# deepqmc/deepqmc

Hardware: AMD Instinct MI355X
Metric: walker*local-energy evals/sec (VMC step: n_sub Metropolis sub-steps + E_loc + energy reduction) (higher is better)
Workload: dtype f32

## Files before the change

deepqmc_amd/csrc/kernel_linear.hip:

```cpp
#include "common.h"
#include "kernels.h"

namespace dqmc {

template <typename real> __device__ __forceinline__ void act_derivs(int act, real v, real& y, real& d1, real& d2) {
  if (act == 1) {
    y = r_tanh<real>(v);
    d1 = 1 - y * y;
    d2 = -2 * y * d1;
  } else if (act == 2) {
    const real s = 1 / (1 + r_exp<real>(-v));
    y = v * s;
    d1 = s * (1 + v * (1 - s));
    d2 = s * (1 - s) * (2 + v * (1 - 2 * s));
  } else if (act == 3) {
    const real av = v < 0 ? -v : v;
    const real e = r_exp<real>(-av);
    const real s = v >= 0 ? 1 / (1 + e) : e / (1 + e);
    y = (v > 0 ? v : (real)0) + (sizeof(real) == 4 ? (real)log1pf((float)e) : (real)log1p((double)e)) - (real)0.69314718055994530942;
    d1 = s;
    d2 = s * (1 - s);
  } else if (act == 4) {
    const real t = r_tanh<real>(v * (real)0.25);
    y = 1 + 2 * t;
// ... 146 lines not shown
        sink.rows(m_ok[q] ? m : 0, drow[q], rrow[q]);
      }
      real rres[2][NR], rpre[2][NR];
#pragma unroll
      for (int q = 0; q < 2; ++q)
#pragma unroll
        for (int n = 0; n < NR; ++n) {
          const int col = col_w0 + n * 16 + cl;
          rres[q][n] = sink.fetch_at(rrow[q], col, col_ok[n] && m_ok[q]);
          rpre[q][n] = (pre != nullptr && col_ok[n]) ? pre[(long)b[q] * ld_pre + col] : (real)0;
        }
#pragma unroll
      for (int q = 0; q < 2; ++q) {
        const int tile_row = wm * (16 * MR) + i * 16 + Mfma<real>::row_of(lane, r0 + q);
#pragma unroll
        for (int n = 0; n < NR; ++n) {
          const int col = col_w0 + n * 16 + cl;
          real v = acc[i][n][r0 + q];
          if (pre != nullptr && col_ok[n]) v += rpre[q][n];
          if (bias != nullptr && col_ok[n]) v += bv[n];
          sink.put_at(drow[q], tile_row, col, act_value<real, ACT>(v), rres[q][n], col_ok[n] && m_ok[q]);
        }
      }
    }
}

template <typename real, int MR, int NR, int GPW, typename Sink>
__device__ __forceinline__ void lin_epilogue(typename Mfma<real>::acc_t (&acc)[MR][NR], const LinArgs<real>& a, const real* bias, int act,
                                             int ldw, const real* pre, int col_w0, int wm, int n_groups, Sink& sink, int bx,
                                             real* xch = nullptr) {
  constexpr bool HALF = GPW == -1;
  constexpr bool SPLIT = GPW == -2;
  constexpr int GB = GPW > 0 ? MR / GPW : 1;
  const int lane = threadIdx.x & 63, cl = lane & 15;
  if (HALF) {
    constexpr bool F32L = sizeof(real) == 4;
    const int wmu = __builtin_amdgcn_readfirstlane(wm);
    const int Tm1 = a.T - 1;
    const int q = lane >> 4;
    real bvh[NR];
    bool col_ok[NR];
#pragma unroll
    for (int n = 0; n < NR; ++n) {
      const int col = col_w0 + n * 16 + cl;
      col_ok[n] = col < ldw;
      bvh[n] = (bias != nullptr && col_ok[n]) ? bias[col] : (real)0;
    }
#pragma unroll
    for (int i = 0; i < MR; ++i) {
      const int g0 = ((bx * 4 + wmu) * MR + i) * 2;
      const bool ok0 = g0 < n_groups, ok1 = g0 + 1 < n_groups;
      if (!ok0) {
        if constexpr (Sink::fills) {
          sink.ugroup2(0, false, col_w0);
#pragma unroll
          for (int n = 0; n < NR; ++n)
#pragma unroll
            for (int rg = 0; rg < 4; ++rg) sink.uput2(false, 0, wm * (16 * MR) + i * 16 + Mfma<real>::row_of(lane, rg), n * 16 + cl, (real)0, (real)0);
        }
        continue;
      }
      sink.ugroup2(g0, ok1, col_w0);
      real rres[NR][4];
#pragma unroll
      for (int n = 0; n < NR; ++n)
#pragma unroll
        for (int rg = 0; rg < 4; ++rg) {
          const int row = Mfma<real>::row_of(lane, rg);
          const bool h = row >> 3;
          rres[n][rg] = (col_ok[n] && (!h || ok1)) ? sink.ufetch2(h, row & 7, n * 16 + cl) : (real)0;
        }
#pragma unroll
      for (int n = 0; n < NR; ++n) {
        real y[2], d1[2], d2S[2];
        if constexpr (F32L) {
          real v = __shfl(acc[i][n][0], (lane & 32) + cl, 64) + bvh[n];
          real s_part = 0;
#pragma unroll
          for (int rg = 0; rg < 4; ++rg) {
            const int tt = (4 * q + rg) & 7;
            const real x = acc[i][n][rg];
            if (tt > 0 && tt < Tm1) s_part += x * x;
          }
          const real S = s_part + __shfl_xor(s_part, 16, 64);
          real d2;
          act_derivs<real>(act, v, y[0], d1[0], d2);
          d2S[0] = d2 * S;
          y[1] = y[0]; d1[1] = d1[0]; d2S[1] = d2S[0];
        } else {
#pragma unroll
          for (int h = 0; h < 2; ++h) {
            const real v = __shfl(acc[i][n][2 * h], cl, 64) + bvh[n];
            real s_part = 0;
#pragma unroll
            for (int rg = 2 * h; rg < 2 * h + 2; ++rg) {
              const int tt = Mfma<real>::row_of(lane, rg) & 7;
              const real x = acc[i][n][rg];
              if (tt > 0 && tt < Tm1) s_part += x * x;
            }
            const real S = quad_sum<real>(s_part);
            real d2;
            act_derivs<real>(act, v, y[h], d1[h], d2);
            d2S[h] = d2 * S;
          }
        }
#pragma unroll
        for (int rg = 0; rg < 4; ++rg) {
          const int row = Mfma<real>::row_of(lane, rg), tt = row & 7;
          const bool h = row >> 3;
          const int hs_ = F32L ? 0 : (rg >> 1);
          const real x = acc[i][n][rg];
          real o = r_fma<real>(d1[hs_], x, tt == Tm1 ? d2S[hs_] : (real)0);
          if (tt == 0) o = y[hs_];
          if (tt > Tm1) o = 0;
          const bool ok = col_ok[n] && (!h || ok1);
          if constexpr (Sink::fills) sink.uput2(h, tt, wm * (16 * MR) + i * 16 + row, n * 16 + cl, ok ? o : (real)0, rres[n][rg]);
          else if (ok) sink.uput2(h, tt, wm * (16 * MR) + i * 16 + row, n * 16 + cl, o, rres[n][rg]);
        }
      }
    }
  } else if (SPLIT) {
    const int half = wm & 1, gl = wm >> 1;
    const int g = bx * 2 + gl;
    const bool g_ok = g < n_groups;
    const int b = (g_ok ? g : 0) / a.nrows;
    const int t0 = half * (16 * MR);
    sink.group(0, g_ok ? g : 0);
    if (pre != nullptr && g_ok) {
#pragma unroll
      for (int n = 0; n < NR; ++n) {
        const int col = col_w0 + n * 16 + cl;
        if (col < ldw) {
#pragma unroll
          for (int tb = 0; tb < MR; ++tb)
#pragma unroll
            for (int rg = 0; rg < 4; ++rg) {
              const int t = t0 + tb * 16 + Mfma<real>::row_of(lane, rg);
              acc[tb][n][rg] += pre[((long)b * a.TP + t) * a.ld_pre + col];
            }
        }
      }
    }
    real* xv = xch + gl * (3 * NR * 16);
    real* xs = xv + NR * 16;
    __syncthreads();
#pragma unroll
    for (int n = 0; n < NR; ++n) {
      real s_part = 0;
#pragma unroll
      for (int tb = 0; tb < MR; ++tb)
#pragma unroll
        for (int rg = 0; rg < 4; ++rg) {
          const int t = t0 + tb * 16 + Mfma<real>::row_of(lane, rg);
          const real x = acc[tb][n][rg];
          if (t >= 1 && t < a.T - 1) s_part += x * x;
        }
      const real Sh = quad_sum<real>(s_part);
      if (lane < 16) {
        xs[half * (NR * 16) + n * 16 + cl] = Sh;
        if (half == 0) xv[n * 16 + cl] = acc[0][n][0];
      }
    }
    __syncthreads();
#pragma unroll
    for (int n = 0; n < NR; ++n) {
      const int col = col_w0 + n * 16 + cl;
      const bool col_ok = col < ldw;
      real v = xv[n * 16 + cl];
      if (bias != nullptr && col_ok) v += bias[col];
      const real S = xs[n * 16 + cl] + xs[NR * 16 + n * 16 + cl];
      real rres[MR][4];
#pragma unroll
      for (int tb = 0; tb < MR; ++tb)
#pragma unroll
        for (int rg = 0; rg < 4; ++rg) rres[tb][rg] = sink.fetch(0, t0 + tb * 16 + Mfma<real>::row_of(lane, rg), col, col_ok && g_ok);
      real y, d1, d2;
      act_derivs<real>(act, v, y, d1, d2);
#pragma unroll
      for (int tb = 0; tb < MR; ++tb)
#pragma unroll
        for (int rg = 0; rg < 4; ++rg) {
          const int row = Mfma<real>::row_of(lane, rg);
          const int t = t0 + tb * 16 + row;
          const real x = acc[tb][n][rg];
          real o;
          if (t == 0) o = y;
          else if (t < a.T - 1) o = d1 * x;
          else if (t == a.T - 1) o = d1 * x + d2 * S;
          else o = 0;
          sink.put(0, t, wm * (16 * MR) + tb * 16 + row, col, o, rres[tb][rg], col_ok && g_ok);
        }
    }
  } else if (GPW > 0) {
    constexpr int NG = GPW > 0 ? GPW : 1;
    constexpr bool HOIST = GB * NR * 4 * (int)(sizeof(real) / 4) <= 32;
    const int wmu = __builtin_amdgcn_readfirstlane(wm);
    const int Tm1 = a.T - 1;
    real bv[NR];
    bool col_ok[NR];
#pragma unroll
    for (int n = 0; n < NR; ++n) {
      const int col = col_w0 + n * 16 + cl;
      col_ok[n] = col < ldw;
      bv[n] = (bias != nullptr && col_ok[n]) ? bias[col] : (real)0;
    }
#pragma unroll
    for (int gj = 0; gj < NG; ++gj) {
      const int g = (bx * 4 + wmu) * GPW + gj;
      if (g >= n_groups) {
        if constexpr (Sink::fills) {
          sink.ugroup(0, col_w0);
#pragma unroll
          for (int n = 0; n < NR; ++n)
#pragma unroll
            for (int tb = 0; tb < GB; ++tb)
#pragma unroll
              for (int rg = 0; rg < 4; ++rg)
                sink.uput(0, wm * (16 * MR) + (gj * GB + tb) * 16 + Mfma<real>::row_of(lane, rg), n * 16 + cl, (real)0, (real)0);
        }
        continue;
      }
      sink.ugroup(g, col_w0);
      if (pre != nullptr) {
        const real* pw = pre + uniform_off((long)(g / a.nrows) * a.TP * a.ld_pre + col_w0);
#pragma unroll
        for (int n = 0; n < NR; ++n) {
          if (col_ok[n]) {
#pragma unroll
            for (int tb = 0; tb < GB; ++tb)
#pragma unroll
              for (int rg = 0; rg < 4; ++rg) {
                const int t = tb * 16 + Mfma<real>::row_of(lane, rg);
                acc[gj * GB + tb][n][rg] += *reinterpret_cast<const real*>(reinterpret_cast<const char*>(pw) + (unsigned)((t * a.ld_pre + n * 16 + cl) * (int)sizeof(real)));
              }
          }
        }
      }
      real rall[HOIST ? NR : 1][HOIST ? GB : 1][4];
      if constexpr (HOIST) {
#pragma unroll
        for (int n = 0; n < NR; ++n)
#pragma unroll
          for (int tb = 0; tb < GB; ++tb)
#pragma unroll
            for (int rg = 0; rg < 4; ++rg)
              rall[n][tb][rg] = col_ok[n] ? sink.ufetch(tb * 16 + Mfma<real>::row_of(lane, rg), n * 16 + cl) : (real)0;
      }
#pragma unroll
      for (int n = 0; n < NR; ++n) {
        real v = __shfl(acc[gj * GB][n][0], cl, 64) + bv[n];
        real s_part = 0;
#pragma unroll
        for (int tb = 0; tb < GB; ++tb)
#pragma unroll
          for (int rg = 0; rg < 4; ++rg) {
            const int t = tb * 16 + Mfma<real>::row_of(lane, rg);
            const real x = acc[gj * GB + tb][n][rg];
            if (t >= 1 && t < Tm1) s_part += x * x;
          }
        const real S = quad_sum<real>(s_part);
        real y, d1, d2;
        act_derivs<real>(act, v, y, d1, d2);
        const real d2S = d2 * S;
        constexpr int FB = HOIST ? GB : (((sizeof(real) == 8 && GB > 2) || GB == 4) ? 2 : GB);
#pragma unroll
        for (int tb0 = 0; tb0 < GB; tb0 += FB) {
          real rres[FB][4];
#pragma unroll
          for (int tb = 0; tb < FB; ++tb)
#pragma unroll
            for (int rg = 0; rg < 4; ++rg) {
              if constexpr (HOIST) rres[tb][rg] = rall[n][tb][rg];
              else rres[tb][rg] = (tb0 + tb < GB && col_ok[n]) ? sink.ufetch((tb0 + tb) * 16 + Mfma<real>::row_of(lane, rg), n * 16 + cl) : (real)0;
            }
          if (Sink::fills || col_ok[n]) {
#pragma unroll
            for (int tb = tb0; tb < tb0 + FB && tb < GB; ++tb)
#pragma unroll
              for (int rg = 0; rg < 4; ++rg) {
                const int row = Mfma<real>::row_of(lane, rg);
                const int t = tb * 16 + row;
                const real x = acc[gj * GB + tb][n][rg];
                real o = r_fma<real>(d1, x, t == Tm1 ? d2S : (real)0);
                if (t == 0) o = y;
                if (t > Tm1) o = 0;
                if (Sink::fills && !col_ok[n]) o = 0;
                sink.uput(t, wm * (16 * MR) + (gj * GB + tb) * 16 + row, n * 16 + cl, o, rres[tb - tb0][rg]);
              }
          }
        }
      }
    }
  } else {
    switch (act) {
      case 1: value_rows_epilogue<real, MR, NR, 1>(acc, a.nrows, a.ld_pre, bias, ldw, pre, col_w0, wm, n_groups, sink, bx); break;
      case 2: value_rows_epilogue<real, MR, NR, 2>(acc, a.nrows, a.ld_pre, bias, ldw, pre, col_w0, wm, n_groups, sink, bx); break;
      case 3: value_rows_epilogue<real, MR, NR, 3>(acc, a.nrows, a.ld_pre, bias, ldw, pre, col_w0, wm, n_groups, sink, bx); break;
      case 4: value_rows_epilogue<real, MR, NR, 4>(acc, a.nrows, a.ld_pre, bias, ldw, pre, col_w0, wm, n_groups, sink, bx); break;
      default: value_rows_epilogue<real, MR, NR, 0>(acc, a.nrows, a.ld_pre, bias, ldw, pre, col_w0, wm, n_groups, sink, bx); break;
    }
  }
}

template <typename real, int MR, int NR, int GPW, int WN, bool CHAIN = false, int NR2 = 2, int BKX = 1>
__global__ void __launch_bounds__(256 * WN, GPW == -2 ? 2 : (GPW == 0 && NR == 4 && WN == 2 && MR * sizeof(real) == 16) ? 4 : 1) k_linear(const LinArgs<real> a) {
  constexpr int NT = 256 * WN;
  constexpr int BM = 64 * MR, BN = 16 * NR * WN, BK = 16 * BKX, BK2 = 16;
  constexpr int AS = BK + 2, BS = BStride<BN>::v;
  constexpr bool HALF = GPW == -1;
  constexpr bool SPLIT = GPW == -2;
  constexpr int GB = GPW > 0 ? MR / GPW : 1;
  constexpr int APT = MR / WN;
  constexpr int NBV = (BK * BN / 4 + NT - 1) / NT;
  constexpr int HS = CHAIN ? BN + 2 : 1;
  constexpr int BN2 = 16 * NR2, BS2 = BStride<BN2>::v;
  constexpr bool FRESH = sizeof(real) == 4 && GPW != 0 && MR <= 3;
  static_assert(MR % WN == 0, "MR must be a multiple of WN");
  static_assert(!CHAIN || WN == 1, "chained layers use one column tile");
  static_assert(!SPLIT || (!CHAIN && WN == 1 && 6 * NR * 16 <= BM * AS), "split groups: plain layers, one column tile per workgroup");
  typedef typename Mfma<real>::acc_t acc_t;
  constexpr int N_AB = BM * AS + BK * BS, N_H = CHAIN ? BM * HS : 0, N_MAIN = N_AB > N_H ? N_AB : N_H;
  __shared__ __attribute__((aligned(32))) real smem_lin[N_MAIN + (CHAIN ? BK2 * BS2 : 0)];
  real* const As = smem_lin;
  real* const Bs = smem_lin + BM * AS;
  real* const Hs = smem_lin;
  real* const Bs2 = smem_lin + N_MAIN;
  static_assert((BM * AS) % 4 == 0 && N_MAIN % 4 == 0, "16-byte (float) / 32-byte (double) aligned LDS tiles");

  const int tid = threadIdx.x, lane = tid & 63, wave = tid >> 6;
  const int wm = wave & 3, wn = wave >> 2;
  const int n_groups = a.B * a.nrows;
  const TileId tile = tile_of_block();
  const int bx = tile.bx;
  const int col_blk0 = tile.by * BN;

  int a_row[APT];
  int a_g[APT], a_t[APT];
  const int a_kq = tid & 3;
#pragma unroll
  for (int j = 0; j < APT; ++j) {
    const int row = (tid >> 2) + (NT / 4) * j;
    a_row[j] = row;
    int g, t;
    if (HALF) {
      const int w = row / (16 * MR), rb = (row >> 4) % MR;
      g = ((bx * 4 + w) * MR + rb) * 2 + ((row & 15) >> 3);
      t = row & 7;
    } else if (SPLIT) {
      const int w = row / (16 * MR), rb = (row >> 4) % MR;
      g = bx * 2 + (w >> 1);
      t = ((w & 1) * MR + rb) * 16 + (row & 15);
    } else if (GPW > 0) {
      const int w = row / (16 * MR), rb = (row >> 4) % MR;
      g = (bx * 4 + w) * GPW + rb / GB;
      t = (rb % GB) * 16 + (row & 15);
    } else {
      g = bx * BM + row;
      t = 0;
    }
    a_g[j] = g < n_groups ? g : -1;
    a_t[j] = t;
  }

  acc_t acc[MR][NR];
#pragma unroll
  for (int i = 0; i < MR; ++i)
#pragma unroll
    for (int j = 0; j < NR; ++j) acc[i][j] = acc_t{0, 0, 0, 0};

  for (int p = 0; p < a.n_pieces; ++p) {
    const LinPiece<real> pc = a.piece[p];
    const int w_row0 = pc.w_row;
    const real* a_src[APT];
#pragma unroll
    for (int j = 0; j < APT; ++j) {
      if (a_g[j] >= 0) {
        const int b = a_g[j] / a.nrows, rr = a_g[j] - b * a.nrows;
        const long srow = ((long)b * pc.rpw + pc.r0 + (pc.bcast ? 0 : rr)) * a.TP + a_t[j];
        a_src[j] = pc.src + srow * pc.ld;
      } else {
        a_src[j] = nullptr;
      }
    }
    const int n_chunks = (pc.K + BK - 1) / BK;
    Vec4<real> ra[APT][BKX];
    real rb_[NBV][4];
    auto load_chunk = [&](int kc) {
#pragma unroll
      for (int j = 0; j < APT; ++j)
#pragma unroll
        for (int x = 0; x < BKX; ++x) {
          const int k0 = kc * BK + 16 * x + 4 * a_kq;
          if (a_src[j] != nullptr && k0 < pc.K) ra[j][x] = *reinterpret_cast<const Vec4<real>*>(a_src[j] + k0);
          else ra[j][x] = Vec4<real>{{0, 0, 0, 0}};
        }
#pragma unroll
      for (int j = 0; j < NBV; ++j) {
        const int f = tid + NT * j;
        const int k = f / (BN / 4), n4 = f % (BN / 4);
        const int kk = kc * BK + k, col = col_blk0 + 4 * n4;
        Vec4<real> t{{0, 0, 0, 0}};
        if (f < BK * BN / 4 && kk < pc.K && col < a.ldw) t = *reinterpret_cast<const Vec4<real>*>(a.W + (long)(w_row0 + kk) * a.ldw + col);
#pragma unroll
        for (int x = 0; x < 4; ++x) rb_[j][x] = t.v[x];
      }
    };
    load_chunk(0);
    for (int kc = 0; kc < n_chunks; ++kc) {
      __syncthreads();
#pragma unroll
      for (int j = 0; j < APT; ++j)
#pragma unroll
        for (int x = 0; x < BKX; ++x) {
          Vec2<real>* dst = reinterpret_cast<Vec2<real>*>(&As[a_row[j] * AS + 16 * x + 4 * a_kq]);
          dst[0] = Vec2<real>{{ra[j][x].v[0], ra[j][x].v[1]}};
          dst[1] = Vec2<real>{{ra[j][x].v[2], ra[j][x].v[3]}};
        }
#pragma unroll
      for (int j = 0; j < NBV; ++j) {
        const int f = tid + NT * j;
        if (f < BK * BN / 4) {
          const int k = f / (BN / 4), n4 = f % (BN / 4);
          *reinterpret_cast<Vec4<real>*>(&Bs[k * BS + 4 * n4]) = Vec4<real>{{rb_[j][0], rb_[j][1], rb_[j][2], rb_[j][3]}};
        }
      }
      __syncthreads();
      if (kc + 1 < n_chunks) load_chunk(kc + 1);
      acc_t part[FRESH ? MR : 1][FRESH ? NR : 1];
      if (FRESH) {
#pragma unroll
        for (int i = 0; i < MR; ++i)
#pragma unroll
          for (int j = 0; j < NR; ++j) part[FRESH ? i : 0][FRESH ? j : 0] = acc_t{0, 0, 0, 0};
      }
#pragma unroll
      for (int kk = 0; kk < BK / 4; ++kk) {
        const int kcol = kk * 4 + (lane >> 4);
        real fa[MR], fb[NR];
#pragma unroll
        for (int i = 0; i < MR; ++i) fa[i] = As[(wm * (16 * MR) + i * 16 + (lane & 15)) * AS + kcol];
#pragma unroll
        for (int j = 0; j < NR; ++j) fb[j] = Bs[kcol * BS + wn * (16 * NR) + j * 16 + (lane & 15)];
#pragma unroll
        for (int i = 0; i < MR; ++i)
#pragma unroll
          for (int j = 0; j < NR; ++j) {
            if (FRESH) part[FRESH ? i : 0][FRESH ? j : 0] = Mfma<real>::run(fa[i], fb[j], part[FRESH ? i : 0][FRESH ? j : 0]);
            else acc[i][j] = Mfma<real>::run(fa[i], fb[j], acc[i][j]);
          }
      }
      if (FRESH) {
#pragma unroll
        for (int i = 0; i < MR; ++i)
#pragma unroll
          for (int j = 0; j < NR; ++j)
#pragma unroll
            for (int x = 0; x < 4; ++x) acc[i][j][x] += part[FRESH ? i : 0][FRESH ? j : 0][x];
      }
    }
  }

  if (!CHAIN) {
    HbmSink<real> sink(a);
    lin_epilogue<real, MR, NR, GPW>(acc, a, a.bias, a.act, a.ldw, a.pre, col_blk0 + wn * (16 * NR), wm, n_groups, sink, bx, As);
    return;
  }
  auto second_layer = [&](acc_t (&h)[MR][NR], const real* bias1, const real* W2, const real* bias2, const LinArgs<real>& out) {
    static_assert(BK2 * BN2 / 4 <= NT, "one W2 vector per thread and chunk");
    const int K2 = a.ldw;
    const int n_chunks2 = (K2 + BK2 - 1) / BK2;
    real w2r[NR][4];
#pragma unroll
    for (int kc = 0; kc < NR; ++kc) {
      const int k = tid / (BN2 / 4), n4 = tid % (BN2 / 4);
      const int kk = kc * BK2 + k, col = 4 * n4;
      Vec4<real> t{{0, 0, 0, 0}};
      if (tid < BK2 * BN2 / 4 && kc < n_chunks2 && kk < K2 && col < a.ldw2) t = *reinterpret_cast<const Vec4<real>*>(W2 + (long)kk * a.ldw2 + col);
#pragma unroll
      for (int x = 0; x < 4; ++x) w2r[kc][x] = t.v[x];
    }
    {
      __syncthreads();
      LdsSink<real> hsink{Hs, HS};
      lin_epilogue<real, MR, NR, GPW>(h, a, bias1, a.act, a.ldw, (const real*)nullptr, 0, wm, n_groups, hsink, bx);
    }
    acc_t acc2[MR][NR2];
#pragma unroll
    for (int i = 0; i < MR; ++i)
#pragma unroll
      for (int j = 0; j < NR2; ++j) acc2[i][j] = acc_t{0, 0, 0, 0};
#pragma unroll
    for (int kc = 0; kc < NR; ++kc) {
      if (kc < n_chunks2) {
      __syncthreads();
      if (tid < BK2 * BN2 / 4) {
        const int k = tid / (BN2 / 4), n4 = tid % (BN2 / 4);
        *reinterpret_cast<Vec4<real>*>(&Bs2[k * BS2 + 4 * n4]) = Vec4<real>{{w2r[kc][0], w2r[kc][1], w2r[kc][2], w2r[kc][3]}};
      }
      __syncthreads();
#pragma unroll
      for (int kk = 0; kk < 4; ++kk) {
        const int kcol = kk * 4 + (lane >> 4);
        real fa[MR], fb[NR2];
#pragma unroll
        for (int i = 0; i < MR; ++i) fa[i] = Hs[(wm * (16 * MR) + i * 16 + (lane & 15)) * HS + kc * BK2 + kcol];
#pragma unroll
        for (int j = 0; j < NR2; ++j) fb[j] = Bs2[kcol * BS2 + j * 16 + (lane & 15)];
#pragma unroll
        for (int i = 0; i < MR; ++i)
#pragma unroll
          for (int j = 0; j < NR2; ++j) acc2[i][j] = Mfma<real>::run(fa[i], fb[j], acc2[i][j]);
      }
      }
    }
    HbmSink<real> sink(out);
    lin_epilogue<real, MR, NR2, GPW>(acc2, out, bias2, a.act2, a.ldw2, (const real*)nullptr, 0, wm, n_groups, sink, bx);
  };
  second_layer(acc, a.bias, a.W2, a.bias2, a);
}

__device__ __forceinline__ void sched_fence() { __builtin_amdgcn_sched_barrier(0); }
template <int MR, int NR, int GPW, int WN, int NP>
__global__ void __launch_bounds__(256 * WN, (MR == 3 && WN == 1) ? 3 : 1) k_linear_bf(const LinArgs<float> a) {
  typedef float real;
  constexpr int NT = 256 * WN;
  constexpr int BM = 64 * MR, BN = 16 * NR * WN, BK = 32;
  constexpr int AS = BK + 2, BSTR = BN + 4;
  constexpr bool HALF = GPW == -1;
  constexpr int GB = GPW > 0 ? MR / GPW : 1;
  constexpr int APT = MR / WN;
  constexpr int NBI = ((BK / 2) * (BN / 4) + NT - 1) / NT;
  constexpr bool HOLD_A = MR <= NR;
  constexpr bool BF_FRESH = NP == 9;
  static_assert(MR % WN == 0, "MR must be a multiple of WN");
  typedef Mfma<float>::acc_t acc_t;
  HIP_DYNAMIC_SHARED(char, smem_raw)
  float* As = reinterpret_cast<float*>(smem_raw);
  uint32_t* Bs = reinterpret_cast<uint32_t*>(smem_raw + (size_t)BM * AS * 4);

  const int tid = threadIdx.x, lane = tid & 63, wave = tid >> 6;
  const int wm = wave & 3, wn = wave >> 2;
  const int n_groups = a.B * a.nrows;
  const TileId tile = tile_of_block();
  const int bx = tile.bx;
  const int col_blk0 = tile.by * BN;
  const int kg = lane >> 4, l15 = lane & 15;

  int a_row[APT], a_g[APT], a_t[APT];
  const int a_kq = tid & 3;
#pragma unroll
  for (int j = 0; j < APT; ++j) {
    const int row = (tid >> 2) + (NT / 4) * j;
    a_row[j] = row;
    int g, t;
    if (HALF) {
      const int w = row / (16 * MR), rb = (row >> 4) % MR;
      g = ((bx * 4 + w) * MR + rb) * 2 + ((row & 15) >> 3);
      t = row & 7;
    } else if (GPW > 0) {
      const int w = row / (16 * MR), rb = (row >> 4) % MR;
      g = (bx * 4 + w) * GPW + rb / GB;
      t = (rb % GB) * 16 + (row & 15);
    } else {
      g = bx * BM + row;
      t = 0;
    }
    a_g[j] = g < n_groups ? g : -1;
    a_t[j] = t;
  }

  acc_t acc[MR][NR];
#pragma unroll
  for (int i = 0; i < MR; ++i)
#pragma unroll
    for (int j = 0; j < NR; ++j) acc[i][j] = acc_t{0, 0, 0, 0};

  for (int p = 0; p < a.n_pieces; ++p) {
    const LinPiece<real> pc = a.piece[p];
    const int w_row0 = pc.w_row;
    const real* a_src[APT];
#pragma unroll
    for (int j = 0; j < APT; ++j) {
      if (a_g[j] >= 0) {
        const int b = a_g[j] / a.nrows, rr = a_g[j] - b * a.nrows;
        const long srow = ((long)b * pc.rpw + pc.r0 + (pc.bcast ? 0 : rr)) * a.TP + a_t[j];
        a_src[j] = pc.src + srow * pc.ld;
      } else {
        a_src[j] = nullptr;
      }
    }
    const int n_chunks = (pc.K + BK - 1) / BK;
    Vec4<real> ra[APT][2], rb_[NBI][2];
    auto load_chunk = [&](int kc) {
#pragma unroll
      for (int j = 0; j < APT; ++j)
#pragma unroll
        for (int x = 0; x < 2; ++x) {
          const int k0 = kc * BK + 16 * x + 4 * a_kq;
          if (a_src[j] != nullptr && k0 < pc.K) ra[j][x] = *reinterpret_cast<const Vec4<real>*>(a_src[j] + k0);
          else ra[j][x] = Vec4<real>{{0, 0, 0, 0}};
        }
#pragma unroll
      for (int j = 0; j < NBI; ++j) {
        const int f = tid + NT * j;
        const int kp = f / (BN / 4), n4 = f % (BN / 4);
        const int kk = kc * BK + 2 * kp, col = col_blk0 + 4 * n4;
#pragma unroll
        for (int h = 0; h < 2; ++h) {
          if (f < (BK / 2) * (BN / 4) && kk + h < pc.K && col < a.ldw)
            rb_[j][h] = *reinterpret_cast<const Vec4<real>*>(a.W + (long)(w_row0 + kk + h) * a.ldw + col);
          else
            rb_[j][h] = Vec4<real>{{0, 0, 0, 0}};
        }
      }
    };
    load_chunk(0);
    for (int kc = 0; kc < n_chunks; ++kc) {
      __syncthreads();
#pragma unroll
      for (int j = 0; j < APT; ++j)
#pragma unroll
        for (int x = 0; x < 2; ++x) {
          Vec2<real>* dst = reinterpret_cast<Vec2<real>*>(&As[a_row[j] * AS + 16 * x + 4 * a_kq]);
          dst[0] = Vec2<real>{{ra[j][x].v[0], ra[j][x].v[1]}};
          dst[1] = Vec2<real>{{ra[j][x].v[2], ra[j][x].v[3]}};
        }
#pragma unroll
      for (int j = 0; j < NBI; ++j) {
        const int f = tid + NT * j;
        if (f < (BK / 2) * (BN / 4)) {
          const int kp = f / (BN / 4), n4 = f % (BN / 4);
          BfFrag* d0 = reinterpret_cast<BfFrag*>(&Bs[(0 * 16 + kp) * BSTR + 4 * n4]);
          BfFrag* d1 = reinterpret_cast<BfFrag*>(&Bs[(1 * 16 + kp) * BSTR + 4 * n4]);
          BfFrag* d2 = reinterpret_cast<BfFrag*>(&Bs[(2 * 16 + kp) * BSTR + 4 * n4]);
          uint32_t w0[4], w1[4], w2[4];
#pragma unroll
          for (int c = 0; c < 4; ++c) {
            const float x0 = rb_[j][0].v[c], x1 = rb_[j][1].v[c];
            const uint32_t h = bf_pack2(x0, x1);
            const float r0 = x0 - bf_lo_as_float(h), r1 = x1 - bf_hi_as_float(h);
            const uint32_t m = bf_pack2(r0, r1);
            w0[c] = h; w1[c] = m; w2[c] = bf_pack2(r0 - bf_lo_as_float(m), r1 - bf_hi_as_float(m));
          }
          *d0 = BfFrag{{w0[0], w0[1], w0[2], w0[3]}};
          *d1 = BfFrag{{w1[0], w1[1], w1[2], w1[3]}};
          *d2 = BfFrag{{w2[0], w2[1], w2[2], w2[3]}};
        }
      }
      __syncthreads();
      if (kc + 1 < n_chunks) load_chunk(kc + 1);
      auto read_a = [&](int i, BfFrag& p0, BfFrag& p1, BfFrag& p2) {
        float av[8];
        const Vec2<real>* src = reinterpret_cast<const Vec2<real>*>(&As[(wm * (16 * MR) + i * 16 + l15) * AS + 8 * kg]);
#pragma unroll
        for (int q = 0; q < 4; ++q) { const Vec2<real> t = src[q]; av[2 * q] = t.v[0]; av[2 * q + 1] = t.v[1]; }
        bf_split8(av, p0, p1, p2);
      };
      auto read_b = [&](int j, BfFrag& p0, BfFrag& p1, BfFrag& p2) {
        const int col = wn * (16 * NR) + j * 16 + l15;
#pragma unroll
        for (int q = 0; q < 4; ++q) {
          p0.w[q] = Bs[(0 * 16 + 4 * kg + q) * BSTR + col];
          p1.w[q] = Bs[(1 * 16 + 4 * kg + q) * BSTR + col];
          p2.w[q] = Bs[(2 * 16 + 4 * kg + q) * BSTR + col];
        }
      };
      if (HOLD_A) {
        BfFrag fa[MR][3];
#pragma unroll
        for (int i = 0; i < MR; ++i) read_a(i, fa[i][0], fa[i][1], fa[i][2]);
#pragma unroll
        for (int j = 0; j < NR; ++j) {
          BfFrag b0, b1, b2;
          read_b(j, b0, b1, b2);
          acc_t part[MR];
#pragma unroll
          for (int i = 0; i < MR; ++i) part[i] = BF_FRESH ? acc_t{0, 0, 0, 0} : acc[i][j];
          if (NP == 9) {
#pragma unroll
            for (int i = 0; i < MR; ++i) part[i] = mfma_bf16(fa[i][2], b2, part[i]);
#pragma unroll
            for (int i = 0; i < MR; ++i) part[i] = mfma_bf16(fa[i][2], b1, part[i]);
#pragma unroll
            for (int i = 0; i < MR; ++i) part[i] = mfma_bf16(fa[i][1], b2, part[i]);
          }
#pragma unroll
          for (int i = 0; i < MR; ++i) part[i] = mfma_bf16(fa[i][2], b0, part[i]);
#pragma unroll
          for (int i = 0; i < MR; ++i) part[i] = mfma_bf16(fa[i][1], b1, part[i]);
#pragma unroll
          for (int i = 0; i < MR; ++i) part[i] = mfma_bf16(fa[i][0], b2, part[i]);
#pragma unroll
          for (int i = 0; i < MR; ++i) part[i] = mfma_bf16(fa[i][1], b0, part[i]);
#pragma unroll
          for (int i = 0; i < MR; ++i) part[i] = mfma_bf16(fa[i][0], b1, part[i]);
#pragma unroll
          for (int i = 0; i < MR; ++i) part[i] = mfma_bf16(fa[i][0], b0, part[i]);
#pragma unroll
          for (int i = 0; i < MR; ++i) {
            if (BF_FRESH) {
#pragma unroll
              for (int x = 0; x < 4; ++x) acc[i][j][x] += part[i][x];
            } else {
              acc[i][j] = part[i];
            }
          }
          sched_fence();
        }
      } else {
        BfFrag fb[NR][3];
#pragma unroll
        for (int j = 0; j < NR; ++j) read_b(j, fb[j][0], fb[j][1], fb[j][2]);
#pragma unroll
        for (int i = 0; i < MR; ++i) {
          BfFrag a0, a1, a2;
          read_a(i, a0, a1, a2);
          acc_t part[NR];
#pragma unroll
          for (int j = 0; j < NR; ++j) part[j] = BF_FRESH ? acc_t{0, 0, 0, 0} : acc[i][j];
          if (NP == 9) {
#pragma unroll
            for (int j = 0; j < NR; ++j) part[j] = mfma_bf16(a2, fb[j][2], part[j]);
#pragma unroll
            for (int j = 0; j < NR; ++j) part[j] = mfma_bf16(a2, fb[j][1], part[j]);
#pragma unroll
            for (int j = 0; j < NR; ++j) part[j] = mfma_bf16(a1, fb[j][2], part[j]);
          }
#pragma unroll
          for (int j = 0; j < NR; ++j) part[j] = mfma_bf16(a2, fb[j][0], part[j]);
#pragma unroll
          for (int j = 0; j < NR; ++j) part[j] = mfma_bf16(a1, fb[j][1], part[j]);
#pragma unroll
          for (int j = 0; j < NR; ++j) part[j] = mfma_bf16(a0, fb[j][2], part[j]);
#pragma unroll
          for (int j = 0; j < NR; ++j) part[j] = mfma_bf16(a1, fb[j][0], part[j]);
#pragma unroll
          for (int j = 0; j < NR; ++j) part[j] = mfma_bf16(a0, fb[j][1], part[j]);
#pragma unroll
          for (int j = 0; j < NR; ++j) part[j] = mfma_bf16(a0, fb[j][0], part[j]);
#pragma unroll
          for (int j = 0; j < NR; ++j) {
            if (BF_FRESH) {
#pragma unroll
              for (int x = 0; x < 4; ++x) acc[i][j][x] += part[j][x];
            } else {
              acc[i][j] = part[j];
            }
          }
          sched_fence();
        }
      }
    }
  }
  HbmSink<real> sink(a);
  lin_epilogue<real, MR, NR, GPW>(acc, a, a.bias, a.act, a.ldw, a.pre, col_blk0 + wn * (16 * NR), wm, n_groups, sink, bx);
}

static bool bf_pays(const LinArgs<float>& a, int np) {
  long chunks = 0, ksteps = 0;
  for (int p = 0; p < a.n_pieces; ++p) { chunks += (a.piece[p].K + 31) / 32; ksteps += (a.piece[p].K + 3) / 4; }
  return a.cfg_bf != 0 && chunks * np * 16 + chunks * 12 < ksteps * 32;
}
template <int MR, int NR, int GPW, int WN> static void launch_bf(hipStream_t st, const LinArgs<float>& a, unsigned gx, unsigned gy) {
  constexpr int BM = 64 * MR, BN = 16 * NR * WN;
  constexpr size_t lds = (size_t)BM * 34 * 4 + (size_t)3 * 16 * (BN + 4) * 4;
  constexpr int NP = GPW == 0 ? 6 : 9;
  static bool attr_set = false;
  if (!attr_set) {
    (void)hipFuncSetAttribute(reinterpret_cast<const void*>(&k_linear_bf<MR, NR, GPW, WN, NP>), hipFuncAttributeMaxDynamicSharedMemorySize, (int)lds);
    attr_set = true;
  }
  hipLaunchKernelGGL(HIP_KERNEL_NAME(k_linear_bf<MR, NR, GPW, WN, NP>), dim3(gx, gy), dim3(256 * WN), lds, st, a);
}
template <typename real, int MR, int NR, int GPW, int WN> struct BfLaunch {
  static bool run(hipStream_t, const LinArgs<real>&, unsigned, unsigned) { return false; }
};
template <int MR, int NR, int GPW, int WN> struct BfLaunch<float, MR, NR, GPW, WN> {
  static bool run(hipStream_t st, const LinArgs<float>& a, unsigned gx, unsigned gy) {
    if (!bf_pays(a, GPW == 0 ? 6 : 9)) return false;
    if (a.cfg_bf >= 2 && !(GPW > 0 && ((MR == 3 && WN == 1) || MR == GPW))) return false;
    launch_bf<MR, NR, GPW, WN>(st, a, gx, gy);
    return true;
  }
};

template <typename real> static bool wide_chunks(const LinArgs<real>& a) {
  int kmax = 0;
  for (int p = 0; p < a.n_pieces; ++p) kmax = a.piece[p].K > kmax ? a.piece[p].K : kmax;
  const bool on = sizeof(real) == 4 ? (a.cfg_bkx == 2 || a.cfg_bkx == 4) : (a.cfg_bkx == 3 || a.cfg_bkx == 4);
  return on && kmax >= 32;
}
template <typename real, int MR, int NR, int GPW, int WN> static void launch_cfg(hipStream_t st, const LinArgs<real>& a) {
  constexpr int BM = 64 * MR, BN = 16 * NR * WN;
  const long n_groups = (long)a.B * a.nrows;
  const unsigned gx = GPW == -2 ? (unsigned)((n_groups + 1) / 2)
                      : GPW < 0 ? (unsigned)((n_groups + 8 * MR - 1) / (8 * MR))
                      : GPW > 0 ? (unsigned)((n_groups + 4 * GPW - 1) / (4 * GPW)) : (unsigned)((n_groups + BM - 1) / BM);
  const unsigned gy = (unsigned)((a.ldw + BN - 1) / BN);
  if (BfLaunch<real, MR, NR, GPW, WN>::run(st, a, gx, gy)) return;
  if (MR == 1 && WN == 1 && GPW != 0 && wide_chunks(a))
    hipLaunchKernelGGL(HIP_KERNEL_NAME(k_linear<real, MR, NR, GPW, WN, false, 2, (MR == 1 && WN == 1 && GPW != 0) ? 2 : 1>), dim3(gx, gy), dim3(256 * WN), 0, st, a);
  else
    hipLaunchKernelGGL(HIP_KERNEL_NAME(k_linear<real, MR, NR, GPW, WN>), dim3(gx, gy), dim3(256 * WN), 0, st, a);
}
template <typename real, int MR, int NR, int GPW, int WN> static void launch_cfg_plain(hipStream_t st, const LinArgs<real>& a) {
  static_assert(GPW > 0 && MR > 1, "one-wave Laplacian groups");
  const long n_groups = (long)a.B * a.nrows;
  const unsigned gx = (unsigned)((n_groups + 4 * GPW - 1) / (4 * GPW)), gy = (unsigned)((a.ldw + 16 * NR * WN - 1) / (16 * NR * WN));
  hipLaunchKernelGGL(HIP_KERNEL_NAME(k_linear<real, MR, NR, GPW, WN>), dim3(gx, gy), dim3(256 * WN), 0, st, a);
}
template <typename real, int MR, int NR, int GPW> static void launch_chain_cfg(hipStream_t st, const LinArgs<real>& a) {
  constexpr int BM = 64 * MR;
  const long n_groups = (long)a.B * a.nrows;
  const unsigned gx = GPW < 0 ? (unsigned)((n_groups + 8 * MR - 1) / (8 * MR))
                      : GPW > 0 ? (unsigned)((n_groups + 4 * GPW - 1) / (4 * GPW)) : (unsigned)((n_groups + BM - 1) / BM);
  if (MR == 1 && GPW != 0 && wide_chunks(a))
    hipLaunchKernelGGL(HIP_KERNEL_NAME(k_linear<real, MR, NR, GPW, 1, true, 2, (MR == 1 && GPW != 0) ? 2 : 1>), dim3(gx, 1), dim3(256), 0, st, a);
  else
    hipLaunchKernelGGL(HIP_KERNEL_NAME(k_linear<real, MR, NR, GPW, 1, true, 2>), dim3(gx, 1), dim3(256), 0, st, a);
}
template <typename real, int MR, int GPW> static void launch_chain_nr(hipStream_t st, const LinArgs<real>& a) {
  if (a.ldw > 32) launch_chain_cfg<real, MR, 4, GPW>(st, a);
  else if (a.ldw > 16) launch_chain_cfg<real, MR, 2, GPW>(st, a);
  else launch_chain_cfg<real, MR, 1, GPW>(st, a);
}
bool linear_chain_supported(int TP, int ldw_hidden, int ldw_out) {
  return (TP == 1 || TP == 8 || TP == 16 || TP == 32) && ldw_hidden <= 64 && ldw_out <= 32;
}
template <typename real> void launch_linear_chain(hipStream_t st, const LinArgs<real>& a) {
  switch (a.TP) {
    case 1: launch_chain_nr<real, 1, 0>(st, a); break;
    case 8: launch_chain_nr<real, 1, -1>(st, a); break;
    case 16: launch_chain_nr<real, 1, 1>(st, a); break;
    case 32: launch_chain_nr<real, 2, 1>(st, a); break;
    default: break;
  }
}

template <typename real, int MR, int GPW> static void launch_nr(hipStream_t st, const LinArgs<real>& a) {
  constexpr int NR_MAX = sizeof(real) == 8 ? 2 : 4;
  constexpr bool WIDE = sizeof(real) == 4 && MR % 2 == 0;
  if (a.ldw > 64 && WIDE) launch_cfg<real, MR, (NR_MAX >= 4 ? 4 : 2), GPW, (WIDE ? 2 : 1)>(st, a);
  else if (a.ldw > 32 && NR_MAX >= 4) launch_cfg<real, MR, (NR_MAX >= 4 ? 4 : 2), GPW, 1>(st, a);
  else if (a.ldw > 16) launch_cfg<real, MR, 2, GPW, 1>(st, a);
  else launch_cfg<real, MR, 1, GPW, 1>(st, a);
}

template <typename real, int MRH> static bool launch_split(hipStream_t st, const LinArgs<real>& a) {
  if constexpr (sizeof(real) == 8) {
    if (!a.cfg_f64_split) return false;
    if (a.ldw > 32) launch_cfg<real, MRH, 4, -2, 1>(st, a);
    else if (a.ldw > 16) launch_cfg<real, MRH, 2, -2, 1>(st, a);
    else launch_cfg<real, MRH, 1, -2, 1>(st, a);
    return true;
  }
  return false;
}

template <typename real, int MR> static void launch_tall(hipStream_t st, const LinArgs<real>& a) {
  if constexpr (sizeof(real) == 4) {
    if (a.ldw > 32) { launch_cfg_plain<real, MR, 4, 1, 1>(st, a); return; }
  }
  launch_cfg_plain<real, MR, 2, 1, 1>(st, a);
}

template <typename real> void launch_linear(hipStream_t st, const LinArgs<real>& a) {
  switch (a.TP) {
    case 1: {
      const long rows = (long)a.B * a.nrows;
      const long col_blocks = (a.ldw + 127) / 128;
      if constexpr (sizeof(real) == 8) {
        if (a.ldw > 64 && (rows + 127) / 128 * col_blocks >= 1024) { launch_cfg<real, 2, 4, 0, 2>(st, a); break; }
      }
      if ((rows + 255) / 256 * col_blocks >= 2048) launch_nr<real, 4, 0>(st, a);
      else if ((rows + 127) / 128 * col_blocks >= 2048) launch_nr<real, 2, 0>(st, a);
      else launch_nr<real, 1, 0>(st, a);
      break;
    }
    case 8: launch_nr<real, 1, -1>(st, a); break;
    case 16: {
      const long wg2 = ((long)a.B * a.nrows + 7) / 8 * ((a.ldw + 127) / 128);
      if (a.ldw > 64 && wg2 >= 256) launch_nr<real, 2, 2>(st, a);
      else launch_nr<real, 1, 1>(st, a);
      break;
    }
    case 32: launch_nr<real, 2, 1>(st, a); break;
    case 48: launch_nr<real, 3, 1>(st, a); break;
    case 64: launch_nr<real, 4, 1>(st, a); break;
    case 80: launch_tall<real, 5>(st, a); break;
    case 96: if (!launch_split<real, 3>(st, a)) launch_nr<real, 6, 1>(st, a); break;
    case 112: launch_tall<real, 7>(st, a); break;
    case 128: if (!launch_split<real, 4>(st, a)) launch_nr<real, 8, 1>(st, a); break;
    case 144: launch_tall<real, 9>(st, a); break;
    case 160: launch_tall<real, 10>(st, a); break;
    case 176: launch_tall<real, 11>(st, a); break;
    case 192: launch_tall<real, 12>(st, a); break;
    case 208: launch_tall<real, 13>(st, a); break;
    default: break;
  }
}

template void launch_linear<float>(hipStream_t, const LinArgs<float>&);
template void launch_linear<double>(hipStream_t, const LinArgs<double>&);
template void launch_linear_chain<float>(hipStream_t, const LinArgs<float>&);
template void launch_linear_chain<double>(hipStream_t, const LinArgs<double>&);

}

#include "kernels_grad.inl"
#include "kernels_jac.inl"
#include "kernels_kfac.inl"
#include "kernels_coords.inl"
#include "kernels_pretrain.inl"
#include "kernels_optim.inl"
#include "kernels_kfacopt.inl"
#include "kernels_loss.inl"
```

Measured before the change: 990,800.

## Flatten piece loop with cross-piece prefetch and unpredicated deferred-mask loads in linear kernels

Restructures the K-loop of the linear and bf16-split linear kernels so that, for selected template instances, the next piece's first chunk is prefetched while the current piece's last chunk computes, removing the pipeline bubble at piece boundaries. Global loads are also issued unconditionally from a safe fallback address, with a validity bitmask applied when staging into LDS. This avoids branchy predicated loads and zero-fills in the load path. Per-instance form selection is hard-coded via template specializations, and one instance gets a higher occupancy hint in launch_bounds. The cost is more live registers across the loop and extra select logic at the LDS store.

New measurement: 981,300. About the same (-1.0%).

```diff
diff --git a/deepqmc_amd/csrc/kernel_linear.hip b/deepqmc_amd/csrc/kernel_linear.hip
--- a/deepqmc_amd/csrc/kernel_linear.hip
+++ b/deepqmc_amd/csrc/kernel_linear.hip
@@ -472,8 +472,28 @@
   }
 }
 
+template <typename real, int MR, int NR, int GPW, int WN, bool CHAIN, int BKX> struct PrefetchForm { static constexpr int v = sizeof(real) == 4 ? 2 : 0; };
+template <int MR, int NR, int GPW, int WN, int NP> struct PrefetchFormBf { static constexpr int v = 2; };
+#define DQMC_PREFETCH_FORM(form, ...) template <> struct PrefetchForm<__VA_ARGS__> { static constexpr int v = form; };
+DQMC_PREFETCH_FORM(1, float, 1, 1, 1, 1, true, 2)
+DQMC_PREFETCH_FORM(1, float, 1, 1, -1, 1, true, 2)
+DQMC_PREFETCH_FORM(1, float, 1, 2, 1, 1, false, 2)
+DQMC_PREFETCH_FORM(1, float, 1, 2, 1, 1, true, 1)
+DQMC_PREFETCH_FORM(1, float, 1, 2, -1, 1, false, 1)
+DQMC_PREFETCH_FORM(1, float, 1, 2, -1, 1, false, 2)
+DQMC_PREFETCH_FORM(1, float, 1, 2, -1, 1, true, 1)
+DQMC_PREFETCH_FORM(1, float, 2, 1, 0, 1, false, 1)
+DQMC_PREFETCH_FORM(1, float, 2, 4, 2, 1, false, 1)
+DQMC_PREFETCH_FORM(1, float, 3, 1, 1, 1, false, 1)
+DQMC_PREFETCH_FORM(1, float, 4, 1, 0, 1, false, 1)
+DQMC_PREFETCH_FORM(1, float, 4, 1, 1, 1, false, 1)
+DQMC_PREFETCH_FORM(0, float, 2, 1, 1, 1, false, 1)
+DQMC_PREFETCH_FORM(0, float, 2, 1, 2, 1, false, 1)
+#undef DQMC_PREFETCH_FORM
+template <> struct PrefetchFormBf<1, 1, -1, 1, 9> { static constexpr int v = 1; };
+template <> struct PrefetchFormBf<8, 4, 1, 2, 9> { static constexpr int v = 0; };
 template <typename real, int MR, int NR, int GPW, int WN, bool CHAIN = false, int NR2 = 2, int BKX = 1>
-__global__ void __launch_bounds__(256 * WN, GPW == -2 ? 2 : (GPW == 0 && NR == 4 && WN == 2 && MR * sizeof(real) == 16) ? 4 : 1) k_linear(const LinArgs<real> a) {
+__global__ void __launch_bounds__(256 * WN, GPW == -2 ? 2 : (GPW == 0 && NR == 4 && WN == 2 && MR * sizeof(real) == 16) ? 4 : (sizeof(real) == 4 && MR == 1 && NR == 2 && GPW == -1 && !CHAIN && BKX == 2) ? 8 : 1) k_linear(const LinArgs<real> a) {
   constexpr int NT = 256 * WN;
   constexpr int BM = 64 * MR, BN = 16 * NR * WN, BK = 16 * BKX, BK2 = 16;
   constexpr int AS = BK + 2, BS = BStride<BN>::v;
@@ -538,10 +558,19 @@
 #pragma unroll
     for (int j = 0; j < NR; ++j) acc[i][j] = acc_t{0, 0, 0, 0};
 
-  for (int p = 0; p < a.n_pieces; ++p) {
-    const LinPiece<real> pc = a.piece[p];
-    const int w_row0 = pc.w_row;
-    const real* a_src[APT];
+  constexpr int FORM = PrefetchForm<real, MR, NR, GPW, WN, CHAIN, BKX>::v;
+  constexpr bool DEFER = FORM >= 1, FLAT = FORM == 2;
+  static_assert(APT * BKX + NBV <= 32, "one predicate bit per prefetched vector");
+  LinPiece<real> pc{};
+  int w_row0 = 0;
+  int n_chunks = 0;
+  const real* a_src[APT];
+  Vec4<real> ra[APT][BKX];
+  real rb_[NBV][4];
+  unsigned ld_ok = 0;
+  auto set_piece = [&](int p) {
+    pc = a.piece[p];
+    w_row0 = pc.w_row;
 #pragma unroll
     for (int j = 0; j < APT; ++j) {
       if (a_g[j] >= 0) {
@@ -552,50 +581,77 @@
         a_src[j] = nullptr;
       }
     }
-    const int n_chunks = (pc.K + BK - 1) / BK;
-    Vec4<real> ra[APT][BKX];
-    real rb_[NBV][4];
-    auto load_chunk = [&](int kc) {
+    n_chunks = (pc.K + BK - 1) / BK;
+  };
+  auto load_chunk = [&](int kc) {
+    unsigned ok_bits = 0;
+#pragma unroll
+    for (int j = 0; j < APT; ++j)
+#pragma unroll
+      for (int x = 0; x < BKX; ++x) {
+        const int k0 = kc * BK + 16 * x + 4 * a_kq;
+        const bool ok = a_src[j] != nullptr && k0 < pc.K;
+        if (DEFER) {
+          ra[j][x] = *reinterpret_cast<const Vec4<real>*>(ok ? a_src[j] + k0 : pc.src);
+          ok_bits |= (unsigned)ok << (j * BKX + x);
+        } else {
+          if (ok) ra[j][x] = *reinterpret_cast<const Vec4<real>*>(a_src[j] + k0);
+          else ra[j][x] = Vec4<real>{{0, 0, 0, 0}};
+        }
+      }
+#pragma unroll
+    for (int j = 0; j < NBV; ++j) {
+      const int f = tid + NT * j;
+      const int k = f / (BN / 4), n4 = f % (BN / 4);
+      const int kk = kc * BK + k, col = col_blk0 + 4 * n4;
+      const bool ok = f < BK * BN / 4 && kk < pc.K && col < a.ldw;
+      Vec4<real> t{{0, 0, 0, 0}};
+      if (DEFER) {
+        t = *reinterpret_cast<const Vec4<real>*>(ok ? a.W + (long)(w_row0 + kk) * a.ldw + col : a.W);
+        ok_bits |= (unsigned)ok << (APT * BKX + j);
+      } else {
+        if (ok) t = *reinterpret_cast<const Vec4<real>*>(a.W + (long)(w_row0 + kk) * a.ldw + col);
+      }
+#pragma unroll
+      for (int x = 0; x < 4; ++x) rb_[j][x] = t.v[x];
+    }
+    ld_ok = ok_bits;
+  };
+  int p = 0;
+  if (FLAT && p < a.n_pieces) { set_piece(p); load_chunk(0); }
+  while (p < a.n_pieces) {
+    if (!FLAT) { set_piece(p); load_chunk(0); }
+    const int nck = n_chunks, pn = p + 1;
+    for (int kc = 0; kc < nck; ++kc) {
+      __syncthreads();
 #pragma unroll
       for (int j = 0; j < APT; ++j)
 #pragma unroll
         for (int x = 0; x < BKX; ++x) {
-          const int k0 = kc * BK + 16 * x + 4 * a_kq;
-          if (a_src[j] != nullptr && k0 < pc.K) ra[j][x] = *reinterpret_cast<const Vec4<real>*>(a_src[j] + k0);
-          else ra[j][x] = Vec4<real>{{0, 0, 0, 0}};
-        }
-#pragma unroll
-      for (int j = 0; j < NBV; ++j) {
-        const int f = tid + NT * j;
-        const int k = f / (BN / 4), n4 = f % (BN / 4);
-        const int kk = kc * BK + k, col = col_blk0 + 4 * n4;
-        Vec4<real> t{{0, 0, 0, 0}};
-        if (f < BK * BN / 4 && kk < pc.K && col < a.ldw) t = *reinterpret_cast<const Vec4<real>*>(a.W + (long)(w_row0 + kk) * a.ldw + col);
-#pragma unroll
-        for (int x = 0; x < 4; ++x) rb_[j][x] = t.v[x];
-      }
-    };
-    load_chunk(0);
-    for (int kc = 0; kc < n_chunks; ++kc) {
-      __syncthreads();
-#pragma unroll
-      for (int j = 0; j < APT; ++j)
-#pragma unroll
-        for (int x = 0; x < BKX; ++x) {
+          const bool ok = !DEFER || ((ld_ok >> (j * BKX + x)) & 1u);
           Vec2<real>* dst = reinterpret_cast<Vec2<real>*>(&As[a_row[j] * AS + 16 * x + 4 * a_kq]);
-          dst[0] = Vec2<real>{{ra[j][x].v[0], ra[j][x].v[1]}};
-          dst[1] = Vec2<real>{{ra[j][x].v[2], ra[j][x].v[3]}};
+          dst[0] = Vec2<real>{{ok ? ra[j][x].v[0] : real(0), ok ? ra[j][x].v[1] : real(0)}};
+          dst[1] = Vec2<real>{{ok ? ra[j][x].v[2] : real(0), ok ? ra[j][x].v[3] : real(0)}};
         }
 #pragma unroll
       for (int j = 0; j < NBV; ++j) {
         const int f = tid + NT * j;
         if (f < BK * BN / 4) {
+          const bool ok = !DEFER || ((ld_ok >> (APT * BKX + j)) & 1u);
           const int k = f / (BN / 4), n4 = f % (BN / 4);
-          *reinterpret_cast<Vec4<real>*>(&Bs[k * BS + 4 * n4]) = Vec4<real>{{rb_[j][0], rb_[j][1], rb_[j][2], rb_[j][3]}};
+          *reinterpret_cast<Vec4<real>*>(&Bs[k * BS + 4 * n4]) =
+              Vec4<real>{{ok ? rb_[j][0] : real(0), ok ? rb_[j][1] : real(0), ok ? rb_[j][2] : real(0), ok ? rb_[j][3] : real(0)}};
         }
       }
       __syncthreads();
-      if (kc + 1 < n_chunks) load_chunk(kc + 1);
+      int kn = kc + 1;
+      bool more = kn < nck;
+      if (FLAT && !more && pn < a.n_pieces) {
+        set_piece(pn);
+        kn = 0;
+        more = true;
+      }
+      if (more) load_chunk(kn);
       acc_t part[FRESH ? MR : 1][FRESH ? NR : 1];
       if (FRESH) {
 #pragma unroll
@@ -628,6 +684,7 @@
             for (int x = 0; x < 4; ++x) acc[i][j][x] += part[FRESH ? i : 0][FRESH ? j : 0][x];
       }
     }
+    p = pn;
   }
 
   if (!CHAIN) {
@@ -745,10 +802,17 @@
 #pragma unroll
     for (int j = 0; j < NR; ++j) acc[i][j] = acc_t{0, 0, 0, 0};
 
-  for (int p = 0; p < a.n_pieces; ++p) {
-    const LinPiece<real> pc = a.piece[p];
-    const int w_row0 = pc.w_row;
-    const real* a_src[APT];
+  constexpr int FORM = PrefetchFormBf<MR, NR, GPW, WN, NP>::v;
+  constexpr bool DEFER = FORM >= 1, FLAT = FORM == 2;
+  static_assert(2 * APT + 2 * NBI <= 32, "one predicate bit per prefetched vector");
+  LinPiece<real> pc{};
+  int w_row0 = 0, n_chunks = 0;
+  const real* a_src[APT];
+  Vec4<real> ra[APT][2], rb_[NBI][2];
+  unsigned ld_ok = 0;
+  auto set_piece = [&](int p) {
+    pc = a.piece[p];
+    w_row0 = pc.w_row;
 #pragma unroll
     for (int j = 0; j < APT; ++j) {
       if (a_g[j] >= 0) {
@@ -759,54 +823,72 @@
         a_src[j] = nullptr;
       }
     }
-    const int n_chunks = (pc.K + BK - 1) / BK;
-    Vec4<real> ra[APT][2], rb_[NBI][2];
-    auto load_chunk = [&](int kc) {
+    n_chunks = (pc.K + BK - 1) / BK;
+  };
+  auto load_chunk = [&](int kc) {
+    unsigned ok_bits = 0;
+#pragma unroll
+    for (int j = 0; j < APT; ++j)
+#pragma unroll
+      for (int x = 0; x < 2; ++x) {
+        const int k0 = kc * BK + 16 * x + 4 * a_kq;
+        const bool ok = a_src[j] != nullptr && k0 < pc.K;
+        if (DEFER) {
+          ra[j][x] = *reinterpret_cast<const Vec4<real>*>(ok ? a_src[j] + k0 : pc.src);
+          ok_bits |= (unsigned)ok << (2 * j + x);
+        } else {
+          if (ok) ra[j][x] = *reinterpret_cast<const Vec4<real>*>(a_src[j] + k0);
+          else ra[j][x] = Vec4<real>{{0, 0, 0, 0}};
+        }
+      }
+#pragma unroll
+    for (int j = 0; j < NBI; ++j) {
+      const int f = tid + NT * j;
+      const int kp = f / (BN / 4), n4 = f % (BN / 4);
+      const int kk = kc * BK + 2 * kp, col = col_blk0 + 4 * n4;
+#pragma unroll
+      for (int h = 0; h < 2; ++h) {
+        const bool ok = f < (BK / 2) * (BN / 4) && kk + h < pc.K && col < a.ldw;
+        if (DEFER) {
+          rb_[j][h] = *reinterpret_cast<const Vec4<real>*>(ok ? a.W + (long)(w_row0 + kk + h) * a.ldw + col : a.W);
+          ok_bits |= (unsigned)ok << (2 * APT + 2 * j + h);
+        } else {
+          if (ok) rb_[j][h] = *reinterpret_cast<const Vec4<real>*>(a.W + (long)(w_row0 + kk + h) * a.ldw + col);
+          else rb_[j][h] = Vec4<real>{{0, 0, 0, 0}};
+        }
+      }
+    }
+    ld_ok = ok_bits;
+  };
+  int p = 0;
+  if (FLAT && p < a.n_pieces) { set_piece(p); load_chunk(0); }
+  while (p < a.n_pieces) {
+    if (!FLAT) { set_piece(p); load_chunk(0); }
+    const int nck = n_chunks, pn = p + 1;
+    for (int kc = 0; kc < nck; ++kc) {
+      __syncthreads();
 #pragma unroll
       for (int j = 0; j < APT; ++j)
 #pragma unroll
         for (int x = 0; x < 2; ++x) {
-          const int k0 = kc * BK + 16 * x + 4 * a_kq;
-          if (a_src[j] != nullptr && k0 < pc.K) ra[j][x] = *reinterpret_cast<const Vec4<real>*>(a_src[j] + k0);
-          else ra[j][x] = Vec4<real>{{0, 0, 0, 0}};
-        }
-#pragma unroll
-      for (int j = 0; j < NBI; ++j) {
-        const int f = tid + NT * j;
-        const int kp = f / (BN / 4), n4 = f % (BN / 4);
-        const int kk = kc * BK + 2 * kp, col = col_blk0 + 4 * n4;
-#pragma unroll
-        for (int h = 0; h < 2; ++h) {
-          if (f < (BK / 2) * (BN / 4) && kk + h < pc.K && col < a.ldw)
-            rb_[j][h] = *reinterpret_cast<const Vec4<real>*>(a.W + (long)(w_row0 + kk + h) * a.ldw + col);
-          else
-            rb_[j][h] = Vec4<real>{{0, 0, 0, 0}};
-        }
-      }
-    };
-    load_chunk(0);
-    for (int kc = 0; kc < n_chunks; ++kc) {
-      __syncthreads();
-#pragma unroll
-      for (int j = 0; j < APT; ++j)
-#pragma unroll
-        for (int x = 0; x < 2; ++x) {
+          const bool ok = !DEFER || ((ld_ok >> (2 * j + x)) & 1u);
           Vec2<real>* dst = reinterpret_cast<Vec2<real>*>(&As[a_row[j] * AS + 16 * x + 4 * a_kq]);
-          dst[0] = Vec2<real>{{ra[j][x].v[0], ra[j][x].v[1]}};
-          dst[1] = Vec2<real>{{ra[j][x].v[2], ra[j][x].v[3]}};
+          dst[0] = Vec2<real>{{ok ? ra[j][x].v[0] : 0.f, ok ? ra[j][x].v[1] : 0.f}};
+          dst[1] = Vec2<real>{{ok ? ra[j][x].v[2] : 0.f, ok ? ra[j][x].v[3] : 0.f}};
         }
 #pragma unroll
       for (int j = 0; j < NBI; ++j) {
         const int f = tid + NT * j;
         if (f < (BK / 2) * (BN / 4)) {
           const int kp = f / (BN / 4), n4 = f % (BN / 4);
+          const bool ok0 = !DEFER || ((ld_ok >> (2 * APT + 2 * j)) & 1u), ok1 = !DEFER || ((ld_ok >> (2 * APT + 2 * j + 1)) & 1u);
           BfFrag* d0 = reinterpret_cast<BfFrag*>(&Bs[(0 * 16 + kp) * BSTR + 4 * n4]);
           BfFrag* d1 = reinterpret_cast<BfFrag*>(&Bs[(1 * 16 + kp) * BSTR + 4 * n4]);
           BfFrag* d2 = reinterpret_cast<BfFrag*>(&Bs[(2 * 16 + kp) * BSTR + 4 * n4]);
           uint32_t w0[4], w1[4], w2[4];
 #pragma unroll
           for (int c = 0; c < 4; ++c) {
-            const float x0 = rb_[j][0].v[c], x1 = rb_[j][1].v[c];
+            const float x0 = ok0 ? rb_[j][0].v[c] : 0.f, x1 = ok1 ? rb_[j][1].v[c] : 0.f;
             const uint32_t h = bf_pack2(x0, x1);
             const float r0 = x0 - bf_lo_as_float(h), r1 = x1 - bf_hi_as_float(h);
             const uint32_t m = bf_pack2(r0, r1);
@@ -818,7 +900,14 @@
         }
       }
       __syncthreads();
-      if (kc + 1 < n_chunks) load_chunk(kc + 1);
+      int kn = kc + 1;
+      bool more = kn < nck;
+      if (FLAT && !more && pn < a.n_pieces) {
+        set_piece(pn);
+        kn = 0;
+        more = true;
+      }
+      if (more) load_chunk(kn);
       auto read_a = [&](int i, BfFrag& p0, BfFrag& p1, BfFrag& p2) {
         float av[8];
         const Vec2<real>* src = reinterpret_cast<const Vec2<real>*>(&As[(wm * (16 * MR) + i * 16 + l15) * AS + 8 * kg]);
@@ -921,11 +1010,15 @@
         }
       }
     }
+    p = pn;
   }
   HbmSink<real> sink(a);
   lin_epilogue<real, MR, NR, GPW>(acc, a, a.bias, a.act, a.ldw, a.pre, col_blk0 + wn * (16 * NR), wm, n_groups, sink, bx);
 }
 
+#ifdef DQMC_LINEAR_ISA_PROBE
+DQMC_LINEAR_ISA_PROBE
+#else
 static bool bf_pays(const LinArgs<float>& a, int np) {
   long chunks = 0, ksteps = 0;
   for (int p = 0; p < a.n_pieces; ++p) { chunks += (a.piece[p].K + 31) / 32; ksteps += (a.piece[p].K + 3) / 4; }
@@ -1075,8 +1168,11 @@
 template void launch_linear_chain<float>(hipStream_t, const LinArgs<float>&);
 template void launch_linear_chain<double>(hipStream_t, const LinArgs<double>&);
 
-}
-
+#endif
+
+}
+
+#ifndef DQMC_LINEAR_ISA_PROBE
 #include "kernels_grad.inl"
 #include "kernels_jac.inl"
 #include "kernels_kfac.inl"
@@ -1085,3 +1181,4 @@
 #include "kernels_optim.inl"
 #include "kernels_kfacopt.inl"
 #include "kernels_loss.inl"
+#endif
```
